# yongduosui/CAL

Measured on AMD Instinct MI355X. Metric: graphs/sec (train step) on SPMotif b=0.9 batch=128, higher is better.
Workload: dtype f32; 1 GPU; spmotif_b0.9_causalgcn_h128_l3_bs128; model=CausalGCN, batch_per_gpu=128, global_batch=128, hidden=128, layers=3, node_num=7, launch=graph(8 steps per graph launch, remainder 3), parallelism=dp1, resident_batches=8

## Files before the change

### cal_amd/csrc/engine.hip

```cpp
#include <string.h>
#include <hip/hip_ext.h>

#include <algorithm>
#include <type_traits>
#include <vector>

#include "engine_kernels.hpp"
#include "engine_readout.hpp"
#include "engine_gconv.hpp"
#include "engine_gconv_bwd.hpp"
#include "engine_ggat.hpp"
#include "engine_plan.hpp"
#include "engine_attbwd.hpp"
#include "engine_ro_step.hpp"
#include "engine_gin.hpp"
#include "engine_ggin.hpp"
#include "engine_feat.hpp"
#include "engine_gwide.hpp"
#include "engine_attwide.hpp"

extern "C" int cal_launch_gconv_bwd_att(unsigned gx, unsigned gy, hipStream_t st, hipEvent_t e0, hipEvent_t e1, const void* csr, size_t csr_bytes,
                                        const int* gptr, const int* eptr, const void* branches, size_t branches_bytes, float loop_w, int N, int H,
                                        int K, int* status, const void* att, size_t att_bytes);

namespace cal {

constexpr int MAX_LAYERS = 6;
constexpr int MAX_SLABS = 24;
constexpr int MAX_COMMITS = 64;

struct FinishArgs {
    SlabTask st[MAX_SLABS];
    CommitTask ct[MAX_COMMITS];
    int nst, nct;
    float* stats;
    float wc, wo, wco;
    float* tick;
    float* ticked;
    unsigned long long* perm_ctr;
    AdamArgs adam;
    AdamRange ar[MAX_ADAM_RANGES];
    int nar;
    double* bn0z; int bn0z_n;
    int* dirty;
    int* host_status;
    const int* status;
    int blk0[MAX_SLABS + MAX_COMMITS + MAX_ADAM_RANGES + 1];
};
__global__ void __launch_bounds__(256) k_finish(const FinishArgs fa, float* __restrict__ grad) {
    int task = 0;
    const int ntask = fa.nst + fa.nct + fa.nar;
    AdamArgs A = fa.adam;
    float adam_t = 0.f, adam_lr = 0.f;
    const bool flagged = fa.status && (fa.status[0] | fa.status[1]) != 0;
    if (fa.ticked && flagged && blockIdx.x == 0 && threadIdx.x == 0) fa.ticked[0] -= 1.f;
    if (A.on && flagged) A.on = 0;
    if (A.on) { adam_t = A.step[0]; adam_lr = A.lr[0]; }
    while (task + 1 < ntask && (int)blockIdx.x >= fa.blk0[task + 1]) ++task;
    const int bx = blockIdx.x - fa.blk0[task], nbx = fa.blk0[task + 1] - fa.blk0[task];
    if (fa.stats && blockIdx.x == 0 && threadIdx.x == 0)
        fa.stats[0] = fa.wc * fa.stats[1] + fa.wo * fa.stats[2] + fa.wco * fa.stats[3];
    if (fa.tick && !flagged && blockIdx.x == 0 && threadIdx.x == 0) fa.tick[0] += 1.f;
    if (fa.perm_ctr && blockIdx.x == 0 && threadIdx.x == 0) fa.perm_ctr[0] += 1;
    if (fa.bn0z && blockIdx.x == 0) {
        for (int i = threadIdx.x; i < fa.bn0z_n; i += 256) fa.bn0z[i] = 0.0;
        if (threadIdx.x == 0) *fa.dirty = 0;
    }
    if (fa.host_status && fa.status && blockIdx.x == 0 && threadIdx.x == 0)
        __hip_atomic_store(fa.host_status, fa.status[0] | fa.status[1], __ATOMIC_RELAXED, __HIP_MEMORY_SCOPE_SYSTEM);
    if (task < fa.nst) {
        const SlabTask t = fa.st[task];
        __shared__ float sred[256];
        const int el = threadIdx.x & 63, grp = threadIdx.x >> 6;
        const int per = (t.S + 3) / 4, z_lo = grp * per, z_hi = min(t.S, z_lo + per);
        for (int i0 = bx * 64; i0 < t.n; i0 += nbx * 64) {
            const int i = min(i0 + el, t.n - 1);
            float s0 = 0.f, s1 = 0.f;
            for (int z0 = z_lo; z0 < z_hi; z0 += 8) {
                float v[8];
#pragma unroll
                for (int u = 0; u < 8; ++u) v[u] = t.slabs[(size_t)max(min(z0 + u, z_hi - 1), 0) * t.n + i];
#pragma unroll
                for (int u = 0; u < 8; ++u) asm volatile("" : "+v"(v[u]));
#pragma unroll
                for (int u = 0; u < 8; u += 2) {
                    s0 += z0 + u < z_hi ? v[u] : 0.f;
                    s1 += z0 + u + 1 < z_hi ? v[u + 1] : 0.f;
                }
            }
            sred[threadIdx.x] = s0 + s1;
            __syncthreads();
            if (grp == 0 && i0 + el < t.n) {
                const float gsum = (sred[el] + sred[64 + el]) + (sred[128 + el] + sred[192 + el]);
                t.dst[i] = gsum;
                if (A.on) adam_update(A, (t.dst - grad) + i, gsum, adam_t, adam_lr);
            }
            __syncthreads();
        }
    } else if (task - fa.nst < fa.nct) {
        const CommitTask t = fa.ct[task - fa.nst];
        __shared__ double red[256];
        const int pl = threadIdx.x >> 4, cl = threadIdx.x & 15;
        for (int c0 = bx * 16; c0 < t.n; c0 += nbx * 16) {
            const int c = c0 + cl, cc = min(c, t.n - 1);
            double sacc = 0.0;
            for (int q0 = pl; q0 < t.P; q0 += 16 * 8) {
// ... 544 lines not shown
    }
    const dim3 grid(cdiv(N, rpb), nbranch);
    if (sd) {
        if (!wt || stt) { set_error("k_espmm: the fused SDDMM is built for the weighted branches without statistics"); return 2; }
        const bool pb = bb.b[0].pb_g != nullptr;
        if (pb != (bb.b[nbranch - 1].pb_g != nullptr)) { set_error("k_espmm: branches differ in kind"); return 2; }
        return with_g(H, [&](auto g) {
            constexpr int G = decltype(g)::value;
            if (pb) PROF_LAUNCH((k_espmm<4, G, true, false, true, true>), grid, dim3(256), 0, st, csr, bb, relu, loop_w, N, H, rpb);
            else PROF_LAUNCH((k_espmm<4, G, true, false, true>), grid, dim3(256), 0, st, csr, bb, relu, loop_w, N, H, rpb);
            return 0;
        });
    }
    return with_g(H, [&](auto g) {
        constexpr int G = decltype(g)::value;
        if (wt && stt) PROF_LAUNCH((k_espmm<4, G, true, true>), grid, dim3(256), 0, st, csr, bb, relu, loop_w, N, H, rpb);
        else if (wt) PROF_LAUNCH((k_espmm<4, G, true, false>), grid, dim3(256), 0, st, csr, bb, relu, loop_w, N, H, rpb);
        else if (stt) PROF_LAUNCH((k_espmm<4, G, false, true>), grid, dim3(256), 0, st, csr, bb, relu, loop_w, N, H, rpb);
        else PROF_LAUNCH((k_espmm<4, G, false, false>), grid, dim3(256), 0, st, csr, bb, relu, loop_w, N, H, rpb);
        return 0;
    });
}

Acc graph_acc(Ctx& c, double* dst, int cols, bool st = false) {
    if (st) return Acc(dst, nullptr, c.e->bn_plane);
    double* p = parts_alloc(c, (size_t)c.T * cols);
    if (!p) return Acc(dst);
    final_task(c, p, c.T, cols, cols, dst);
    return Acc(dst, p, cols);
}
CSR csr_dst(const Ctx& c) { return CSR{c.e->rowptr_dst, c.e->nbr_dst, c.e->eid_dst, (int)c.E}; }
CSR csr_src(const Ctx& c) { return CSR{c.e->rowptr_src, c.e->nbr_src, c.e->eid_src, (int)c.E}; }

template <typename Args>
int bn_bwd_sums(Ctx& c, Args& a, int P, double* dsum, double* dprod, bool st) {
    if (st) { a.dacc_sum = dsum; a.dacc_prod = dprod; a.dacc_ss = c.e->bn_plane; return 0; }
    const int H = c.e->H;
    double* p = parts_alloc(c, (size_t)P * 2 * H);
    if (!p) return no_parts();
    a.dot_parts = p;
    final_task(c, p, P, 2 * H, H, dsum);
    final_task(c, p + H, P, 2 * H, H, dprod);
    return 0;
}

int gconv_bwd(Ctx& c, Bwd& b, GconvBwdBranch* gb, int nb, float** dst, double** dsum, double** dprod, bool st, const AttBwdGraphArgs* att = nullptr) {
    Engine* e = c.e;
    const bool co = nb == 2;
    const bool wide = (co ? c.r.co_bwd : c.r.bb_bwd) == Conv::Wide;
    const int nsplit = co ? c.r.nsplit_co : c.r.nsplit_bb;
    const bool lean = co ? c.r.lean_co : c.r.lean_bb;
    const int H = e->H, B = c.T, nsl = H / GC_N;
    const int np2 = nsplit == 4 ? 2 : 1;
    for (int k = 0; k < nb; ++k) {
        gb[k].batch = c.batch; gb[k].tile_gptr = e->ntiles > 0 ? e->tile_gptr : nullptr;
        RCP(gb[k].slab = b.slabs(c, B, H * H, dst[k]));
        RC(bn_bwd_sums(c, gb[k], B * nsl * np2, dsum[k], dprod[k], st));
    }
    const GconvBwdBranch2 b2{{gb[0], gb[nb - 1]}};
    if (wide) {
        const CSR gs = csr_src(c);
        const dim3 gridw(B, nsl * nsplit, nb);
        if (co) PROF_LAUNCH((k_gw_bwd<true, 2>), gridw, dim3(GW_NT), 0, c.st, gs, e->gptr, e->eptr, b2, e->loop_w, c.N, H, H, nsplit, e->status);
        else if (gb[0].dout) PROF_LAUNCH((k_gw_bwd<false, 0>), gridw, dim3(GW_NT), 0, c.st, gs, e->gptr, e->eptr, b2, e->loop_w, c.N, H, H, nsplit, e->status);
        else PROF_LAUNCH((k_gw_bwd<false, 1>), gridw, dim3(GW_NT), 0, c.st, gs, e->gptr, e->eptr, b2, e->loop_w, c.N, H, H, nsplit, e->status);
        CAL_CHECK_LAUNCH("k_gw_bwd");
        return 0;
    }
    const CSR gd = csr_dst(c);
    const dim3 grid(B, nsl, nb);
    if (att) {
        if (co || lean || gb[0].dout) { set_error("k_gconv_bwd: the ATT mode is a one-branch, one-workgroup-per-CU launch"); return 2; }
        if (cal_launch_gconv_bwd_att(grid.x, grid.y, c.st, g_prof_cur ? g_prof_cur->r.e0 : nullptr, g_prof_cur ? g_prof_cur->r.e1 : nullptr, &gd, sizeof(gd),
                                     e->gptr, e->eptr, &b2, sizeof(b2), e->loop_w, c.N, H, H, e->status, att, sizeof(*att))) {
            set_error("k_gconv_bwd_att: argument structures differ between engine.hip and gconv_bwd_att.hip"); return 2;
        }
        if (g_prof_cur) g_prof_cur->used = true;
        CAL_CHECK_LAUNCH("k_att_bwd_graph");
        return 0;
    }
    const bool tiles = e->ntiles > 0;
    auto kern = co ? (lean ? (tiles ? k_gconv_bwd<true, 2, true, true> : k_gconv_bwd<true, 2, false, true>) : tiles ? k_gconv_bwd<true, 2, true> : k_gconv_bwd<true, 2>)
              : gb[0].dout ? (lean ? k_gconv_bwd<false, 0, false, true> : k_gconv_bwd<false, 0>) : lean ? k_gconv_bwd<false, 1, false, true> : k_gconv_bwd<false, 1>;
    PROF_LAUNCH(kern, grid, dim3(GB_NT), 0, c.st, gd, e->gptr, e->eptr, b2, e->loop_w, c.N, H, H, e->status);
    CAL_CHECK_LAUNCH("k_gconv_bwd");
    return 0;
}

RoArgs make_ro(const Ctx& c) {
    Engine* e = c.e;
    const int L = e->L, H = e->H, C = e->C, B = c.B;
    RoArgs a;
    memset(&a, 0, sizeof(a));
    for (int hd = 0; hd < 3; ++hd) {
        RoHead& h = a.h[hd];
        const int k1 = L + 3 + 2 * hd, k2 = L + 4 + 2 * hd;
        h.W1 = e->P + e->o_fc1_w[hd]; h.b1 = e->P + e->o_fc1_b[hd];
        h.W2 = e->P + e->o_fc2_w[hd]; h.b2 = e->P + e->o_fc2_b[hd];
        h.bn1 = bnref(c, k1, B, 1); h.bn2 = bnref(c, k2, B, 1);
        h.st2_sum = bn_stsum(c, k2); h.st2_sq = bn_stsq(c, k2);
        h.d1_sum = bn_dsum(c, k1); h.d1_prod = bn_dprod(c, k1);
        h.d2_sum = bn_dsum(c, k2); h.d2_prod = bn_dprod(c, k2);
        h.db1 = e->arena + e->a_db1 + hd * H; h.db2 = e->arena + e->a_db2 + hd * C;
        h.gW1 = e->G + e->o_fc1_w[hd]; h.gW2 = e->G + e->o_fc2_w[hd];
    }
    a.pooled = e->pooled; a.perm = c.perm; a.iperm = e->iperm; a.xco = e->xco; a.y1 = e->y1;
    a.zl = e->zl; a.logp = e->logp; a.dzl = e->dzl; a.dy1 = e->dy1; a.dxin = e->dxh;
    a.rowloss = e->dyh1;
    a.y = c.y; a.stats = e->stats; a.B = B; a.H = H; a.C = C;
    a.wc = c.wc; a.wo = c.wo; a.wco = c.wco; a.training = c.training; a.want_grad = c.want_grad;
    return a;
}

static int g_stop_after = 0;
static int g_stage = 0;
static std::vector<const char*> g_stage_names;
#define STAGE() do { if (g_stop_after == 0) g_stage_names.push_back(cal::g_last_launch); \
                     if (g_stop_after > 0 && ++g_stage >= g_stop_after) return -12345; } while (0)

int gin_rows(Ctx& c, int mode, const GinRowArgs& ga) {
    const int N = c.N, H = c.e->H;
    hipStream_t st = c.st;
    return with_g(H, [&](auto g) {
        constexpr int G = decltype(g)::value;
        const dim3 grid(cdiv(N, c.rpb_n));
        if (mode == 0) hipLaunchKernelGGL((k_gin_rows<4, G, 0>), grid, dim3(256), 0, st, ga, N, H, c.rpb_n);
        else if (mode == 1) hipLaunchKernelGGL((k_gin_rows<4, G, 1>), grid, dim3(256), 0, st, ga, N, H, c.rpb_n);
        else if (mode == 2) hipLaunchKernelGGL((k_gin_rows<4, G, 2>), grid, dim3(256), 0, st, ga, N, H, c.rpb_n);
        else hipLaunchKernelGGL((k_gin_rows<4, G, 3>), grid, dim3(256), 0, st, ga, N, H, c.rpb_n);
        return 0;
    });
}

template <typename Fn>
int with_g_fp(int H, int F, Fn f) {
    return with_g(H, [&](auto g) {
        constexpr int G = decltype(g)::value;
        if constexpr (G >= FEAT_FMAX) {
            if (F <= 4) return f(g, std::integral_constant<int, 4>());
            if (F <= 8) return f(g, std::integral_constant<int, 8>());
            if (F <= 12) return f(g, std::integral_constant<int, 12>());
            return f(g, std::integral_constant<int, 16>());
        } else {
            set_error("feature row kernels: hidden width too small"); return 2;
        }
    });
}

int pool2_slices(int N, int B) { return std::max(1, std::min(32, N / std::max(1, B * 128))); }
int launch_pool2(hipStream_t st, const float* hc, const float* ho, const int* gptr, float* pooled, float* cnt, float* slices,
                 int N, int B, int H) {
    const int tc = std::min(256, pow2ceil(H / 4));
    const int S = pool2_slices(N, B);
    hipLaunchKernelGGL((k_pool2<4>), dim3(B, 2, S), dim3(256), 0, st, hc, ho, gptr, pooled, pooled + (size_t)B * H, H, tc, slices, cnt);
    CAL_CHECK_LAUNCH("k_pool2");
    if (S > 1) {
        hipLaunchKernelGGL(k_pool2_sum, dim3(cdiv(4 * (int64_t)B * H, 256)), dim3(256), 0, st, slices, S, 2 * (int64_t)B * H, pooled, cnt);
        CAL_CHECK_LAUNCH("k_pool2_sum");
    }
    return 0;
}
int launch_pool2(Ctx& c) {
    Engine* e = c.e;
    const size_t NH = (size_t)c.N * e->H;
    return launch_pool2(c.st, e->hco, e->hco + NH, e->gptr, e->pooled, e->pcnt, e->dZco, (int)c.N, (int)c.B, e->H);
}
// ... 1218 lines not shown
    CAL_REQUIRE(e != nullptr && max_nodes >= 0 && max_edges >= 0, "bad arguments");
    e->max_nodes = (int)std::min<int64_t>(max_nodes, 1 << 30);
    e->max_edges = (int)std::min<int64_t>(max_edges, 1 << 30);
    return 0;
}
CAL_EXPORT int cal_engine_set_graph_ptrs(void* h, const int64_t* node_ptr, const int64_t* edge_ptr) {
    Engine* e = (Engine*)h;
    CAL_REQUIRE(e != nullptr, "bad arguments");
    e->node_ptr = node_ptr; e->edge_ptr = edge_ptr;
    return 0;
}
CAL_EXPORT int cal_engine_set_tiles(void* h, const int64_t* tile_gptr, int64_t ntiles) {
    Engine* e = (Engine*)h;
    CAL_REQUIRE(e != nullptr && ntiles >= 0 && (ntiles == 0 || tile_gptr != nullptr), "bad arguments");
    e->tile_gptr = ntiles > 0 ? tile_gptr : nullptr; e->ntiles = (int)ntiles;
    return 0;
}
CAL_EXPORT int cal_engine_set_deterministic(void* h, int on) {
    Engine* e = (Engine*)h;
    CAL_REQUIRE(e != nullptr, "bad arguments");
    e->striped = on ? 0 : 1;
    return 0;
}
CAL_EXPORT int cal_engine_debug_stop(int k) { g_stop_after = k; return 0; }
CAL_EXPORT const char* cal_engine_stage_name(int k) {
    return k >= 1 && k <= (int)g_stage_names.size() ? g_stage_names[k - 1] : "";
}

CAL_EXPORT int cal_sparse_probe_espmm(const int64_t* iv, void* const* pv, const double* dv, void* stream_) {
    CAL_REQUIRE(iv && pv && dv, "description missing");
    const int64_t nnz = iv[0], nbranch = iv[1], N = iv[3], H = iv[4], rpb = iv[5];
    CAL_REQUIRE(nbranch == 1 || nbranch == 2, "one or two branches");
    CAL_REQUIRE(H % 4 == 0 && H >= 4 && H <= 256, "hidden must be a multiple of 4 in [4, 256]");
    CAL_REQUIRE(N >= 1 && N < (1ll << 31) && nnz >= 0 && nnz < (1ll << 31) && rpb >= 1 && rpb < (1ll << 31), "sizes out of range");
    CSR csr;
    csr.ptr = (const int*)pv[0]; csr.nbr = (const int*)pv[1]; csr.eid = (const int*)pv[2]; csr.nnz = (int)nnz;
    SpmmBranch2 bb;
    for (int b = 0; b < 2; ++b) {
        const int64_t* ib = iv + 6 + 2 * std::min<int64_t>(b, nbranch - 1);
        void* const* pb = pv + 3 + 14 * std::min<int64_t>(b, nbranch - 1);
        SpmmBranch& br = bb.b[b];
        br.h = (const float*)pb[0]; br.out = (float*)pb[1]; br.bias = (const float*)pb[2]; br.w = (const float*)pb[3];
        br.dis = (const float*)pb[4];
        br.st_sum = Acc((double*)pb[5], (double*)pb[6], (int)ib[0]);
        br.st_sq = Acc((double*)pb[7], (double*)pb[8], (int)ib[1]);
        br.sd_z = (const float*)pb[9]; br.sd_gn = (float*)pb[10]; br.sd_gself = (float*)pb[11];
        br.pb_g = (const float*)pb[12]; br.pb_batch = (const int64_t*)pb[13];
    }
    RC(launch_espmm((hipStream_t)stream_, csr, bb, (int)nbranch, (int)iv[2], (float)dv[0], (int)N, (int)H, (int)rpb));
    CAL_CHECK_LAUNCH("k_espmm(probe)");
    return 0;
}
CAL_EXPORT int cal_sparse_probe_edge_att(const int* ptr, const int* nbr, const int* eid, int64_t nnz, const float* pq, const float* be,
                                         float* att, float* dis_c, float* dis_o, double loop_w, int64_t N, int64_t E, double fedge,
                                         void* stream_) {
    CAL_REQUIRE(ptr && nbr && eid && pq && be && att && dis_c && dis_o, "null argument");
    CAL_REQUIRE(N >= 1 && N < (1ll << 31) && E >= 0 && nnz >= 0 && nnz < (1ll << 31), "sizes out of range");
    CSR gs;
    gs.ptr = ptr; gs.nbr = nbr; gs.eid = eid; gs.nnz = (int)nnz;
    hipLaunchKernelGGL(k_edge_att_deg, dim3(cdiv(N, 32)), dim3(256), 0, (hipStream_t)stream_, gs, pq, be, att, dis_c, dis_o,
                       (float)loop_w, (int)N, E, (float)fedge);
    CAL_CHECK_LAUNCH("k_edge_att_deg(probe)");
    return 0;
}
CAL_EXPORT int cal_sparse_probe_pool(int sel, const float* hc, const float* ho, const int* gptr, const int64_t* batch, float* pooled,
                                     float* cnt, float* slices, int64_t N, int64_t B, int64_t H, int64_t rpb_n, int64_t* S_out,
                                     void* stream_) {
    CAL_REQUIRE(sel >= 0 && sel <= 3 && S_out != nullptr, "bad selector");
    CAL_REQUIRE(H % 4 == 0 && H >= 4 && H <= 256, "hidden must be a multiple of 4 in [4, 256]");
    CAL_REQUIRE(N >= 1 && N < (1ll << 31) && B >= 1 && B < (1ll << 31), "sizes out of range");
    const int S = pool2_slices((int)N, (int)B);
    *S_out = S;
    if (sel == 3) return 0;
    CAL_REQUIRE(hc && ho && (sel == 2 ? batch != nullptr && cnt != nullptr && rpb_n >= 1 && rpb_n < (1ll << 31) : gptr != nullptr && pooled != nullptr),
                "null argument");
    if (sel == 2) return launch_pool_cnt((hipStream_t)stream_, hc, ho, batch, cnt, (int)N, (int)B, (int)H, (int)rpb_n);
    CAL_REQUIRE(S == 1 || slices != nullptr, "row slices without a slice buffer");
    return launch_pool2((hipStream_t)stream_, hc, ho, gptr, pooled, sel == 0 ? cnt : nullptr, slices, (int)N, (int)B, (int)H);
}
#ifdef CAL_BLK_CLOCKS
CAL_EXPORT int cal_debug_blk_clocks(long long* out) {
    return (int)hipMemcpyFromSymbol(out, HIP_SYMBOL(cal::g_blk_clk), sizeof(long long) * 8192);
}
#endif
#ifdef CAL_RO_CLOCKS
CAL_EXPORT int cal_debug_ro_clocks(long long* out) {
    return (int)hipMemcpyFromSymbol(out, HIP_SYMBOL(cal::g_ro_clk), sizeof(long long) * 64);
}
#endif

CAL_EXPORT int cal_engine_profile(int on) {
    g_prof_on = on != 0;
    if (on) {
        for (auto& r : g_prof) { hipEventDestroy(r.e0); hipEventDestroy(r.e1); }
        g_prof.clear();
    }
    return 0;
}
CAL_EXPORT int64_t cal_engine_profile_read(double* out, int64_t cap) {
    int64_t n = 0;
    for (auto& r : g_prof) {
        if (n >= cap) break;
        float ms = 0.f;
        if (hipEventElapsedTime(&ms, r.e0, r.e1) != hipSuccess) ms = -1.f;
        out[3 * n] = r.cls; out[3 * n + 1] = ms; out[3 * n + 2] = r.work;
        ++n;
    }
    return n;
}

CAL_EXPORT int cal_engine_adam(void* h, void* stream_) {
    Engine* e = (Engine*)h;
    hipStream_t st = (hipStream_t)stream_;
    RC(launch_adam(e, st, 0));
    hipLaunchKernelGGL(k_adam_tick, dim3(1), dim3(1), 0, st, e->step);
    CAL_CHECK_LAUNCH("k_adam_tick");
    return 0;
}
CAL_EXPORT int cal_engine_adam_ticked(void* h, void* stream_) {
    return launch_adam((Engine*)h, (hipStream_t)stream_, 1);
}
CAL_EXPORT int cal_p2p_alloc(int64_t bytes, void** out) {
    CAL_REQUIRE(bytes > 0 && out, "bad arguments");
    void* p = nullptr;
    hipError_t rc = hipExtMallocWithFlags(&p, (size_t)bytes, hipDeviceMallocFinegrained);
    if (rc != hipSuccess || !p) { (void)hipGetLastError(); set_error("cal_p2p_alloc: hipExtMallocWithFlags(fine-grained, %lld bytes): %s", (long long)bytes, hipGetErrorString(rc)); return 3; }
    rc = hipMemset(p, 0, (size_t)bytes);
    if (rc == hipSuccess) rc = hipDeviceSynchronize();
    if (rc != hipSuccess) { (void)hipGetLastError(); (void)hipFree(p); set_error("cal_p2p_alloc: zeroing failed: %s", hipGetErrorString(rc)); return 3; }
    *out = p;
    return 0;
}
CAL_EXPORT int cal_p2p_free(void* p) {
    if (p && hipFree(p) != hipSuccess) { (void)hipGetLastError(); set_error("cal_p2p_free failed"); return 3; }
    return 0;
}
CAL_EXPORT int cal_p2p_export(void* p, void* handle64) {
    CAL_REQUIRE(p && handle64, "bad arguments");
    static_assert(sizeof(hipIpcMemHandle_t) == 64, "IPC handle size");
    hipIpcMemHandle_t hd;
    hipError_t rc = hipIpcGetMemHandle(&hd, p);
    if (rc != hipSuccess) { (void)hipGetLastError(); set_error("cal_p2p_export: hipIpcGetMemHandle: %s", hipGetErrorString(rc)); return 3; }
    memcpy(handle64, &hd, 64);
    return 0;
}
CAL_EXPORT int cal_p2p_open(const void* handle64, void** out) {
    CAL_REQUIRE(handle64 && out, "bad arguments");
    hipIpcMemHandle_t hd;
    memcpy(&hd, handle64, 64);
    void* p = nullptr;
    hipError_t rc = hipIpcOpenMemHandle(&p, hd, hipIpcMemLazyEnablePeerAccess);
    if (rc != hipSuccess || !p) { (void)hipGetLastError(); set_error("cal_p2p_open: hipIpcOpenMemHandle: %s", hipGetErrorString(rc)); return 3; }
    *out = p;
    return 0;
}
CAL_EXPORT int cal_p2p_close(void* p) {
    if (p && hipIpcCloseMemHandle(p) != hipSuccess) { (void)hipGetLastError(); set_error("cal_p2p_close failed"); return 3; }
    return 0;
}
CAL_EXPORT int64_t cal_engine_p2p_region_bytes(void* h) {
    Engine* e = (Engine*)h;
    const int64_t np = (e->nparam + 63) / 64 * 64;
    return (2 * np + 64) * 4;
}
CAL_EXPORT int cal_engine_p2p_bind(void* h, void* const* peer_bases, const int64_t* peer_devices, int64_t world, int64_t rank) {
    Engine* e = (Engine*)h;
// ... 79 lines not shown
```

### cal_amd/csrc/engine_gconv_bwd.hpp

```cpp
#pragma once
#include "engine_gconv.hpp"
#include "engine_attphases.hpp"

namespace cal {

constexpr int GB_NT = 512;
constexpr int GB_T = 64;
constexpr int GB_E = 1024;
constexpr int GB_LDJ = GB_T + 1;
constexpr int GB_LDD = GC_N + 4;
constexpr int GB_LDW = GC_K + 1;
constexpr int GB_LDX = GC_K + 4;

struct GconvBwdBranch {
    const float* dout;
    const float* x;
    const float* W;
    const float* ew;
    const float* dis;
    const float* rs;
    int rs_stride;
    BNRef bn;
    float* dxp0; float* dxp1;
    float* slab;
    double* dot_parts;
    double* dacc_sum; double* dacc_prod; int dacc_ss;
    const float* coef_in;
    const float* dy0; const float* dy1;
    const float* y;
    BNRef ubn;
    const double* udot_sum; const double* udot_prod;
    double* bias_parts;
    const float* gp0; const float* gp1; const int* iperm;
    const float* z;
    float* gn; float* gself;
    size_t gn_stride, gself_stride;
    int gn_slot;
    const int64_t* batch;
    const int64_t* tile_gptr;
};

struct GconvBwdBranch2 { GconvBwdBranch b[2]; };
struct GconvBwdNoAtt {};
template <int MODE> struct GconvBwdNoAttOf { using type = GconvBwdNoAtt; };

template <bool RS, int MODE, bool TILED = false, bool LEAN = false>
__global__ void __launch_bounds__(GB_NT, (LEAN ? 4 : 1)) k_gconv_bwd(const CSR g, const int* __restrict__ gptr, const int* __restrict__ eptr,
                                                   const GconvBwdBranch2 bb, float loop_w, int N, int H,
                                                   int K, int* __restrict__ status) {
    static_assert(MODE != 3, "the ATT mode is the kernel k_gconv_bwd_att (gconv_bwd_att.hip)");
    [[maybe_unused]] const typename GconvBwdNoAttOf<MODE>::type ga{};
#include "engine_gconv_bwd_body.hpp"
}

constexpr int FB_T = 64, FB_F = 64, FB_H = 128;
struct FeatBwdArgs {
    const float* dy0; const float* dy1;
    const float* y;
    BNRef ubn; const double* udot_sum; const double* udot_prod;
    const float* x0;
    const float* W;
    BNRef bn0;
    float* slab;
    double* parts;
};
template <int FMAX>
__global__ void __launch_bounds__(GB_NT) k_feat_bwd(const int* __restrict__ gptr, const FeatBwdArgs a, int H, int F,
                                                  int* __restrict__ status, int N) {
    __shared__ __attribute__((aligned(16))) float Dz[FB_T * (FB_H + 4)];
    __shared__ float Xn[FB_T * FMAX];
    __shared__ __attribute__((aligned(16))) float Ws[FMAX * (FB_H + 4)];
    __shared__ float um_s[FB_H], ur_s[FB_H], ug_s[FB_H], u1_s[FB_H], u2_s[FB_H];
    __shared__ float m0_s[FMAX], r0_s[FMAX], g0_s[FMAX], b0_s[FMAX];
    __shared__ float dX0[FB_T * FMAX];
    BLK_CLK(0);
    warm_kernargs<sizeof(FeatBwdArgs) + 32>();
    const int b = blockIdx.x, t = threadIdx.x, LDZ = FB_H + 4;
    const int g0 = gptr ? gptr[b] : b * FB_T, rows = gptr ? gptr[b + 1] - g0 : min(FB_T, N - g0);
    float* slab = a.slab + (size_t)b * F * H;
    double* parts = a.parts + (size_t)b * 2 * F;
    if (rows <= 0 || rows > FB_T) {
        if (rows > 0 && t == 0) atomicOr(status, 8);
        for (int i = t; i < F * H; i += GB_NT) slab[i] = 0.f;
        for (int i = t; i < 2 * F; i += GB_NT) parts[i] = 0.0;
        return;
    }
    const int H4 = H >> 2;
// ... 300 lines not shown
```

### cal_amd/csrc/engine_gconv_bwd_body.hpp

```cpp
    constexpr int LDX = LEAN ? GC_K : GB_LDX;
    __shared__ __attribute__((aligned(16))) float Ab[GB_T * GB_LDJ];
    __shared__ __attribute__((aligned(16))) float Ds[GB_T * GB_LDD];
    __shared__ __attribute__((aligned(16))) float Ws[LEAN ? 4 : GC_K * GB_LDD];
    __shared__ __attribute__((aligned(16))) float Xs[GB_T * LDX];
    __shared__ float mean_s[GC_K], rstd_s[GC_K], gam_s[GC_K], bet_s[GC_K];
    __shared__ int ptr_s[GB_T + 4];
    __shared__ float dis_s[GB_T], rs_s[GB_T];
    __shared__ unsigned char en[GB_E];
    __shared__ float ec[GB_E];
    __shared__ float um_s[MODE == 1 ? GC_N : 1], ur_s[MODE == 1 ? GC_N : 1], ug_s[MODE == 1 ? GC_N : 1], u1_s[MODE == 1 ? GC_N : 1], u2_s[MODE == 1 ? GC_N : 1];
    __shared__ float bs_s[GB_NT / 64][16][4];
    __shared__ __attribute__((aligned(16))) float Zr_own[(MODE == 2 && !LEAN) ? GB_T * GB_LDD : 4];
    float* const Zr = (MODE == 2 && LEAN) ? Xs : Zr_own;
    __shared__ float gv_s[TILED ? GC_TILE_GRAPHS * GC_N : GC_N];
    __shared__ unsigned char bg_s[TILED ? GB_T : 4];
    __shared__ int ee[(MODE == 2 && !LEAN) ? GB_E : 1];
    __shared__ unsigned char er[GB_E];
    constexpr bool UP = MODE == 1, POOL = MODE == 2, ATT = MODE == 3;
    static_assert(!TILED || MODE == 2, "only the POOL variant looks at the graphs inside a tile");
    static_assert(!ATT || (!LEAN && !RS), "the ATT mode keeps the staged W slice (one workgroup per CU) and has no row scales");
    __shared__ double red[ATT ? 8 : 1][4][ATT ? GC_N : 1];
    __shared__ double sc_lds[2][ATT ? 8 : 1];
    __shared__ float bnk_s[ATT ? 8 : 1][ATT ? GC_K : 1];
    __shared__ float dis_c_s[ATT ? GB_T : 1], dis_o_s[ATT ? GB_T : 1], dd_c_s[ATT ? GB_T : 1], dd_o_s[ATT ? GB_T : 1], spv_s[ATT ? GB_T : 1], sqv_s[ATT ? GB_T : 1],
// ... 281 lines not shown
        float cs[4] = {0.f, 0.f, 0.f, 0.f};
        const bool two = br.dy1 != nullptr;
#pragma unroll
        for (int u = 0; u < 2; ++u) { ro_pin(bd.v[u]); ro_pin(bd1.v[u]); ro_pin(by.v[u]); }
        const int c = 4 * (t & 15);
#pragma unroll
        for (int u = 0; u < 2; ++u) {
            const int j = (t >> 4) + u * (GB_NT / 16);
            if (j < rows) {
                const float4 v0 = bd.v[u], v1 = bd1.v[u], yv = by.v[u];
                const float d[4] = {v0.x + (two ? v1.x : 0.f), v0.y + (two ? v1.y : 0.f), v0.z + (two ? v1.z : 0.f), v0.w + (two ? v1.w : 0.f)};
                const float yy[4] = {yv.x, yv.y, yv.z, yv.w};
                float o[4];
#pragma unroll
                for (int q = 0; q < 4; ++q) {
                    const float yn = (yy[q] - um_s[c + q]) * ur_s[c + q];
                    const float g1 = ug_s[c + q] * (d[q] - u1_s[c + q] - yn * u2_s[c + q]);
                    o[q] = yy[q] > 0.f ? g1 : 0.f;
                    cs[q] += o[q];
                }
                *reinterpret_cast<float4*>(Ds + j * GB_LDD + c) = make_float4(o[0], o[1], o[2], o[3]);
            }
        }
#pragma unroll
        for (int q = 0; q < 4; ++q) {
            cs[q] += __shfl_xor(cs[q], 16, 64);
            cs[q] += __shfl_xor(cs[q], 32, 64);
        }
        if (lane < 16) {
#pragma unroll
            for (int q = 0; q < 4; ++q) bs_s[t >> 6][lane][q] = cs[q];
        }
    }
    for (int i = t; i < (rowsP - rows) * GB_LDD; i += GB_NT) Ds[rows * GB_LDD + i] = 0.f;
    for (int i = t; i < (rowsP - rows) * LDX; i += GB_NT) Xs[rows * LDX + i] = 0.f;
    if (!ATT) adj_scatter<GB_NT, GB_LDJ>(Ab, er, en, un, t, [&](int j, int s) { return dis_s[j] * ec[s]; }, [&](int j) { return dis_s[j] * dis_s[j] * loop_w; });
    __syncthreads();
    if ((UP || POOL) && t < GC_N) {
        double tot = 0.0;
#pragma unroll
        for (int k = 0; k < GB_NT / 64; ++k) tot += (double)bs_s[k][t >> 2][t & 3];
        br.bias_parts[(size_t)b * H + ns0 + t] = tot;
    }
    if (!ATT) BLK_CLK(2); else BLK_CLK_W(3, 0, t);
    auto ident = [](float v) { return v; };
    gc_f32x16 acc[2];
    {
        const int rt = w >> 1, ct = w & 1;
#pragma unroll
        for (int i = 0; i < 16; ++i) { acc[0][i] = 0.f; acc[1][i] = 0.f; }
        if (rt < R) mma_kmajor<1, 1, GB_LDJ, GB_LDD>(Ab + rt * 32 + li, Ds + ct * 32 + li, rowsP, lk, ident, MmaIdent(), acc);
        if constexpr (ATT) { if (w >= 4) att_colsum_store(ga.a, red, sc_lds, t - 256, 256, ns0, GC_N, H, sl == 0); }
        if (POOL && w >= 4) {
            const int q4 = (t - 256) & 3, it0 = (t - 256) >> 2;
            float* gn = br.gn + (size_t)sl * br.gn_stride;
            float* gs = br.gself + (size_t)sl * br.gself_stride;
            for (int it = it0; it - it0 < ne + rows; it += 64) {
                const bool ok = it < ne + rows, isedge = it < ne;
                const int itc = ok ? it : 0;
                const int jd = isedge ? er[itc] : itc - ne, js = isedge ? en[itc] : itc - ne;
                const float4* a = reinterpret_cast<const float4*>(Ds + (ok ? jd : 0) * GB_LDD + 16 * q4);
                const float4* bsrc = reinterpret_cast<const float4*>(Zr + (ok ? js : 0) * GB_LDD + 16 * q4);
                float p = 0.f;
#pragma unroll
                for (int k = 0; k < 4; ++k) p = dot4(a[k], bsrc[k], p);
                p += __shfl_xor(p, 1, 64);
                p += __shfl_xor(p, 2, 64);
                if (ok && q4 == 0) {
                    if (isedge) gn[(LEAN || br.gn_slot) ? e0 + itc : ee[itc]] = p; else gs[g0 + itc - ne] = p;
                }
            }
        }
        __syncthreads();
        if (POOL && LEAN) commit_x();
        if (rt < R) {
#pragma unroll
            for (int r = 0; r < 16; ++r) {
                const int row = mma_row(r, lk, rt * 32);
                Ds[row * GB_LDD + ct * 32 + li] = acc[0][r];
            }
        }
        __syncthreads();
    }
    if (w < 4 && w * 32 < K) {
#pragma unroll
        for (int i = 0; i < 16; ++i) { acc[0][i] = 0.f; acc[1][i] = 0.f; }
        const float* wrow = LEAN ? br.W + (size_t)min(w * 32 + li, K - 1) * H + ns0 : Ws + (w * 32 + li) * GB_LDD;
        if (R == 2) mma_rowk<true>(Ds + li * GB_LDD, Ds + (32 + li) * GB_LDD, wrow, GC_N, lk, acc[0], acc[1]);
        else mma_rowk<false>(Ds + li * GB_LDD, nullptr, wrow, GC_N, lk, acc[0], acc[1]);
        const int k = w * 32 + li;
        float* dxp = sl ? br.dxp1 : br.dxp0;
        float xh[2][16];
#pragma unroll
        for (int q = 0; q < 2; ++q)
#pragma unroll
            for (int r = 0; r < 16; ++r) xh[q][r] = Xs[(mma_row(r, lk, q * 32)) * LDX + k];
#pragma unroll
        for (int q = 0; q < 2; ++q)
#pragma unroll
            for (int r = 0; r < 16; ++r) { asm volatile("" : "+v"(xh[q][r])); if (q >= R) xh[q][r] = 0.f; }
        float f1[4] = {0.f, 0.f, 0.f, 0.f}, f2[4] = {0.f, 0.f, 0.f, 0.f};
#pragma unroll
        for (int q = 0; q < 2; ++q) {
#pragma unroll
            for (int r = 0; r < 16; ++r) {
                const int i = mma_row(r, lk, q * 32);
                const float v = acc[q][r];
                f1[r & 3] += v;
                f2[r & 3] = fmaf(v, xh[q][r], f2[r & 3]);
            }
        }
        gc_store_tile<gc_site(WT_DXP)>(acc[0], dxp + (size_t)g0 * K + w * 32, K, rows, li, lk, MmaIdent(), (rows * K - w * 32) * 4);
        if (R == 2) gc_store_tile<gc_site(WT_DXP)>(acc[1], dxp + (size_t)(g0 + 32) * K + w * 32, K, rows - 32, li, lk, MmaIdent(), ((rows - 32) * K - w * 32) * 4);
        double s1, s2;
        colsum_fold(f1, f2, s1, s2);
        if (lk == 0) {
            if (br.dacc_sum) {
                const size_t po = (size_t)stripe_of_block() * br.dacc_ss + k;
                atomicAdd(br.dacc_sum + po, s1); atomicAdd(br.dacc_prod + po, s2);
            } else { parts[k] = s1; parts[K + k] = s2; }
        }
    }
    if (!ATT) BLK_CLK(3);
    if (w >= 4 && (w - 4) * 32 < K) {
        const int wq = w - 4, k = wq * 32 + li;
        const float gam = gam_s[k], bet = bet_s[k];
        auto affine = [&](float v) { return fmaf(v, gam, bet); };
#pragma unroll
        for (int i = 0; i < 16; ++i) { acc[0][i] = 0.f; acc[1][i] = 0.f; }
        mma_kmajor<1, 2, LDX, GB_LDD>(Xs + wq * 32 + li, Ds + li, rowsP, lk, affine, MmaIdent(), acc);
#pragma unroll
        for (int q = 0; q < 2; ++q) {
            const int off = wq * 32 * H + ns0 + q * 32;
            gc_store_tile<gc_site(WT_DW)>(acc[q], slab + off, H, 32, li, lk, MmaIdent(), (K * H - off) * 4);
        }
    }
    BLK_CLK(1);
```

### cal_amd/csrc/engine_kernels.hpp

```cpp
#pragma once
#include "engine.hpp"

namespace cal {

#ifdef CAL_BLK_CLOCKS
__device__ long long g_blk_clk[4 * 2048];
#define BLK_CLK(which) do { const int b_ = blockIdx.x + gridDim.x * blockIdx.y; \
                            if (threadIdx.x == 0 && b_ < 2048) g_blk_clk[4 * b_ + ((which) == 1 ? 3 : (which) == 0 ? 0 : (which) - 1)] = wall_clock64(); } while (0)
#define BLK_CLK_W(which, wv, dep) do { const int b_ = blockIdx.x + gridDim.x * blockIdx.y; int d_; \
                            asm volatile("s_waitcnt vmcnt(0) lgkmcnt(0)\n\tv_readfirstlane_b32 %0, %1" : "=s"(d_) : "v"(dep)); \
                            if ((int)threadIdx.x == 64 * (wv) && b_ < 2048) g_blk_clk[4 * b_ + ((which) == 1 ? 3 : (which) == 0 ? 0 : (which) - 1)] = wall_clock64() + (d_ & 0); } while (0)
#else
#define BLK_CLK(which) do {} while (0)
#define BLK_CLK_W(which, wv, dep) do {} while (0)
#endif

struct CSR {
    const int* ptr;
    const int* nbr;
    const int* eid;
    int nnz;
};

struct Acc {
    double* dst;
    double* parts;
    int stride;
    __host__ __device__ Acc() : dst(nullptr), parts(nullptr), stride(0) {}
    __host__ __device__ Acc(double* d) : dst(d), parts(nullptr), stride(0) {}
    __host__ __device__ Acc(double* d, double* p, int s) : dst(d), parts(p), stride(s) {}
    __host__ __device__ bool on() const { return dst != nullptr || parts != nullptr; }
    __device__ __forceinline__ void add(int col, double t) const {
        if (parts) parts[(size_t)blockIdx.x * stride + col] = t;
        else atomicAdd(dst + (size_t)stripe_of_block() * stride + col, t);
    }
};

__device__ __forceinline__ void block_col_atomic(double v, int cslot, int rlane, int nrl, int ncols, bool valid,
                                                 const Acc& dst, int col, double* lds) {
    lds[rlane * ncols + cslot] = valid ? v : 0.0;
    __syncthreads();
    if (rlane == 0 && valid) {
        double t = 0.0;
        for (int k = 0; k < nrl; ++k) t += lds[k * ncols + cslot];
        dst.add(col, t);
    }
    __syncthreads();
}

template <int NV>
__device__ __forceinline__ void block_col_sums(const double (&v)[NV], int cslot, int rlane, int nrl, int ncols, bool valid,
                                               double* lds, double (&out)[NV]) {
#pragma unroll
    for (int q = 0; q < NV; ++q) lds[(q * nrl + rlane) * ncols + cslot] = valid ? v[q] : 0.0;
    __syncthreads();
    if (rlane == 0 && valid) {
#pragma unroll
        for (int q = 0; q < NV; ++q) {
            double t = 0.0;
            for (int k = 0; k < nrl; ++k) t += lds[(q * nrl + k) * ncols + cslot];
            out[q] = t;
        }
    }
    __syncthreads();
}

struct FinalTask { const double* parts; int P; int stride; int n; double* dst; };
struct FinalArgs { FinalTask t[8]; int nt; };
__global__ void __launch_bounds__(256) k_stats_final(const FinalArgs fa) {
    __shared__ double red[256];
    const FinalTask t = fa.t[blockIdx.y];
    const int c = blockIdx.x * 8 + (threadIdx.x & 7), pl = threadIdx.x >> 3;
    const int cc = min(c, t.n - 1);
    double s0 = 0.0, s1 = 0.0;
    for (int p0 = pl; p0 < t.P; p0 += 32 * 8) {
        double v[8];
#pragma unroll
        for (int u = 0; u < 8; ++u) v[u] = t.parts[(size_t)min(p0 + 32 * u, t.P - 1) * t.stride + cc];
#pragma unroll
        for (int u = 0; u < 8; ++u) asm volatile("" : "+v"(v[u]));
#pragma unroll
        for (int u = 0; u < 8; u += 2) {
            s0 += p0 + 32 * u < t.P ? v[u] : 0.0;
            s1 += p0 + 32 * (u + 1) < t.P ? v[u + 1] : 0.0;
        }
    }
    red[threadIdx.x] = s0 + s1;
    __syncthreads();
    if (pl == 0 && c < t.n) {
        double tot = 0.0;
#pragma unroll
        for (int k = 0; k < 32; ++k) tot += red[k * 8 + (threadIdx.x & 7)];
        t.dst[c] = tot;
    }
}

constexpr int ZP_CAP = 1024;
// ... 1168 lines not shown
```

### cal_amd/csrc/gconv_bwd_att.hip

```cpp
#include <hip/hip_runtime.h>
#include <hip/hip_ext.h>
#include <stdint.h>
#include <string.h>

namespace {
#include "engine_kernels.hpp"
#include "engine_readout.hpp"
#include "engine_gconv.hpp"
#include "engine_gconv_bwd.hpp"
#include "engine_attbwd.hpp"

namespace cal {
__global__ void __launch_bounds__(GB_NT, 1) k_gconv_bwd_att(const CSR g, const int* __restrict__ gptr, const int* __restrict__ eptr,
                                                           const GconvBwdBranch2 bb, float loop_w, int N, int H,
                                                           int K, int* __restrict__ status, const AttBwdGraphArgs ga) {
    constexpr bool RS = false, TILED = false, LEAN = false;
    constexpr int MODE = 3;
#include "engine_gconv_bwd_body.hpp"
}
}
}

extern "C" int cal_launch_gconv_bwd_att(unsigned gx, unsigned gy, hipStream_t st, hipEvent_t e0, hipEvent_t e1, const void* csr, size_t csr_bytes,
                                        const int* gptr, const int* eptr, const void* branches, size_t branches_bytes, float loop_w, int N, int H,
                                        int K, int* status, const void* att, size_t att_bytes) {
    using namespace cal;
    if (csr_bytes != sizeof(CSR) || branches_bytes != sizeof(GconvBwdBranch2) || att_bytes != sizeof(AttBwdGraphArgs)) return 2;
    CSR g; GconvBwdBranch2 bb; AttBwdGraphArgs ga;
    memcpy(&g, csr, sizeof(g)); memcpy(&bb, branches, sizeof(bb)); memcpy(&ga, att, sizeof(ga));
    const dim3 grid(gx, gy, 1);
    if (e0) hipExtLaunchKernelGGL(k_gconv_bwd_att, grid, dim3(GB_NT), 0, st, e0, e1, 0, g, gptr, eptr, bb, loop_w, N, H, K, status, ga);
    else hipLaunchKernelGGL(k_gconv_bwd_att, grid, dim3(GB_NT), 0, st, g, gptr, eptr, bb, loop_w, N, H, K, status, ga);
    return 0;
}
```

Before: 619,500 graphs/s.

## Split gconv backward dX work across all waves and run dW after

Adds a sequential variant of the gconv backward tail. All eight waves now compute the dX tiles, each wave taking one row tile and one 32-column slice, and the two row-tile halves of the column sums are combined through LDS. The dW tiles are then computed in a second phase, replacing the old split where waves 0-3 did dX and waves 4-7 did dW concurrently. The variant is compiled in a separate translation unit and selected by default (CAL_GCB_ORDER=1) for the non-lean instantiations. It also adds extra clock instrumentation macros for timing each phase.

```diff
diff --git a/cal_amd/csrc/engine.hip b/cal_amd/csrc/engine.hip
--- a/cal_amd/csrc/engine.hip
+++ b/cal_amd/csrc/engine.hip
@@ -22,6 +22,9 @@
 extern "C" int cal_launch_gconv_bwd_att(unsigned gx, unsigned gy, hipStream_t st, hipEvent_t e0, hipEvent_t e1, const void* csr, size_t csr_bytes,
                                         const int* gptr, const int* eptr, const void* branches, size_t branches_bytes, float loop_w, int N, int H,
                                         int K, int* status, const void* att, size_t att_bytes);
+extern "C" int cal_launch_gconv_bwd_seq(int sel, unsigned gx, unsigned gy, unsigned gz, hipStream_t st, hipEvent_t e0, hipEvent_t e1, const void* csr,
+                                        size_t csr_bytes, const int* gptr, const int* eptr, const void* branches, size_t branches_bytes, float loop_w,
+                                        int N, int H, int K, int* status);
 
 namespace cal {
 
@@ -732,6 +735,15 @@
     const bool tiles = e->ntiles > 0;
     auto kern = co ? (lean ? (tiles ? k_gconv_bwd<true, 2, true, true> : k_gconv_bwd<true, 2, false, true>) : tiles ? k_gconv_bwd<true, 2, true> : k_gconv_bwd<true, 2>)
               : gb[0].dout ? (lean ? k_gconv_bwd<false, 0, false, true> : k_gconv_bwd<false, 0>) : lean ? k_gconv_bwd<false, 1, false, true> : k_gconv_bwd<false, 1>;
+    if (CAL_GCB_ORDER != 0 && (!lean || CAL_GCB_ORDER == 2)) {
+        const int sel = (co ? 1 : 0) | (co && tiles ? 2 : 0) | (!co && gb[0].dout ? 4 : 0) | (lean ? 8 : 0);
+        const int rc = cal_launch_gconv_bwd_seq(sel, grid.x, grid.y, grid.z, c.st, g_prof_cur ? g_prof_cur->r.e0 : nullptr, g_prof_cur ? g_prof_cur->r.e1 : nullptr,
+                                                &gd, sizeof(gd), e->gptr, e->eptr, &b2, sizeof(b2), e->loop_w, c.N, H, H, e->status);
+        if (rc) { set_error(rc == 2 ? "k_gconv_bwd: argument structures differ between engine.hip and gconv_bwd_seq.hip" : "k_gconv_bwd: instantiation missing from gconv_bwd_seq.hip"); return 2; }
+        if (g_prof_cur) g_prof_cur->used = true;
+        CAL_CHECK_LAUNCH("k_gconv_bwd");
+        return 0;
+    }
     PROF_LAUNCH(kern, grid, dim3(GB_NT), 0, c.st, gd, e->gptr, e->eptr, b2, e->loop_w, c.N, H, H, e->status);
     CAL_CHECK_LAUNCH("k_gconv_bwd");
     return 0;
@@ -2116,6 +2128,9 @@
 CAL_EXPORT int cal_debug_blk_clocks(long long* out) {
     return (int)hipMemcpyFromSymbol(out, HIP_SYMBOL(cal::g_blk_clk), sizeof(long long) * 8192);
 }
+CAL_EXPORT int cal_debug_blk_clocks_x(long long* out) {
+    return (int)hipMemcpyFromSymbol(out, HIP_SYMBOL(cal::g_blk_clk_x), sizeof(long long) * 8192);
+}
 #endif
 #ifdef CAL_RO_CLOCKS
 CAL_EXPORT int cal_debug_ro_clocks(long long* out) {
diff --git a/cal_amd/csrc/engine_gconv_bwd.hpp b/cal_amd/csrc/engine_gconv_bwd.hpp
--- a/cal_amd/csrc/engine_gconv_bwd.hpp
+++ b/cal_amd/csrc/engine_gconv_bwd.hpp
@@ -3,6 +3,15 @@
 #include "engine_attphases.hpp"
 
 namespace cal {
+
+#ifndef CAL_GCB_ORDER
+#define CAL_GCB_ORDER 1
+#endif
+#ifdef CAL_GCB_UNIT
+constexpr bool GCB_SEQ = CAL_GCB_ORDER != 0, GCB_SEQ_LEAN = CAL_GCB_ORDER == 2;
+#else
+constexpr bool GCB_SEQ = false, GCB_SEQ_LEAN = false;
+#endif
 
 constexpr int GB_NT = 512;
 constexpr int GB_T = 64;
diff --git a/cal_amd/csrc/engine_gconv_bwd_body.hpp b/cal_amd/csrc/engine_gconv_bwd_body.hpp
--- a/cal_amd/csrc/engine_gconv_bwd_body.hpp
+++ b/cal_amd/csrc/engine_gconv_bwd_body.hpp
@@ -387,12 +387,72 @@
         }
         __syncthreads();
     }
+    constexpr bool SEQ = GCB_SEQ && (!LEAN || GCB_SEQ_LEAN);
+    if constexpr (SEQ) {
+    {
+        const int rt = w >> 2, kq = w & 3, k = kq * 32 + li;
+        const bool on = kq * 32 < K;
+        float4* const park = reinterpret_cast<float4*>(Ab);
+        float xh[16];
+        float f1[4] = {0.f, 0.f, 0.f, 0.f}, f2[4] = {0.f, 0.f, 0.f, 0.f};
+#pragma unroll
+        for (int i = 0; i < 16; ++i) acc[0][i] = 0.f;
+        if (on) {
+            const float* wrow = LEAN ? br.W + (size_t)k * H + ns0 : Ws + k * GB_LDD;
+            if (rt < R) mma_rowk(Ds + (rt * 32 + li) * GB_LDD, wrow, GC_N, lk, acc[0]);
+            BLK_CLK_X(4, 4, acc[0][15]);
+#pragma unroll
+            for (int r = 0; r < 16; ++r) xh[r] = Xs[(mma_row(r, lk, rt * 32)) * LDX + k];
+#pragma unroll
+            for (int r = 0; r < 16; ++r) { asm volatile("" : "+v"(xh[r])); if (rt >= R) xh[r] = 0.f; }
+            float* dxp = sl ? br.dxp1 : br.dxp0;
+            if (rt < R) gc_store_tile<gc_site(WT_DXP)>(acc[0], dxp + (size_t)(g0 + rt * 32) * K + kq * 32, K, rows - rt * 32, li, lk, MmaIdent(),
+                                                       ((rows - rt * 32) * K - kq * 32) * 4);
+            if (rt == 0) {
+#pragma unroll
+                for (int r = 0; r < 16; ++r) { const float v = acc[0][r]; f1[r & 3] += v; f2[r & 3] = fmaf(v, xh[r], f2[r & 3]); }
+                park[(2 * kq) * 64 + lane] = make_float4(f1[0], f1[1], f1[2], f1[3]);
+                park[(2 * kq + 1) * 64 + lane] = make_float4(f2[0], f2[1], f2[2], f2[3]);
+            }
+        }
+        __syncthreads();
+        if (!ATT) BLK_CLK(3);
+        if (on && rt == 1) {
+            const float4 p1 = park[(2 * kq) * 64 + lane], p2 = park[(2 * kq + 1) * 64 + lane];
+            f1[0] = p1.x; f1[1] = p1.y; f1[2] = p1.z; f1[3] = p1.w;
+            f2[0] = p2.x; f2[1] = p2.y; f2[2] = p2.z; f2[3] = p2.w;
+#pragma unroll
+            for (int r = 0; r < 16; ++r) { const float v = acc[0][r]; f1[r & 3] += v; f2[r & 3] = fmaf(v, xh[r], f2[r & 3]); }
+            double s1, s2;
+            colsum_fold(f1, f2, s1, s2);
+            if (lk == 0) {
+                if (br.dacc_sum) {
+                    const size_t po = (size_t)stripe_of_block() * br.dacc_ss + k;
+                    atomicAdd(br.dacc_sum + po, s1); atomicAdd(br.dacc_prod + po, s2);
+                } else { parts[k] = s1; parts[K + k] = s2; }
+            }
+        }
+        BLK_CLK_X(5, 4, f1[0]);
+    }
+    if (w < (K >> 4)) {
+        const int ct = w >= (K >> 5) ? 1 : 0, kt = w - ct * (K >> 5), k = kt * 32 + li;
+        const float gam = gam_s[k], bet = bet_s[k];
+        auto affine = [&](float v) { return fmaf(v, gam, bet); };
+#pragma unroll
+        for (int i = 0; i < 16; ++i) acc[0][i] = 0.f;
+        mma_kmajor_ptrs<1, 1, LDX, GB_LDD>(Xs + kt * 32 + li, nullptr, Ds + ct * 32 + li, nullptr, rowsP, lk, affine, MmaIdent(), acc);
+        const int off = kt * 32 * H + ns0 + ct * 32;
+        gc_store_tile<gc_site(WT_DW)>(acc[0], slab + off, H, 32, li, lk, MmaIdent(), (K * H - off) * 4);
+    }
+    BLK_CLK_X(6, 4, acc[0][15]);
+    } else {
     if (w < 4 && w * 32 < K) {
 #pragma unroll
         for (int i = 0; i < 16; ++i) { acc[0][i] = 0.f; acc[1][i] = 0.f; }
         const float* wrow = LEAN ? br.W + (size_t)min(w * 32 + li, K - 1) * H + ns0 : Ws + (w * 32 + li) * GB_LDD;
         if (R == 2) mma_rowk<true>(Ds + li * GB_LDD, Ds + (32 + li) * GB_LDD, wrow, GC_N, lk, acc[0], acc[1]);
         else mma_rowk<false>(Ds + li * GB_LDD, nullptr, wrow, GC_N, lk, acc[0], acc[1]);
+        BLK_CLK_X(4, 0, acc[0][15]);
         const int k = w * 32 + li;
         float* dxp = sl ? br.dxp1 : br.dxp0;
         float xh[2][16];
@@ -425,6 +485,7 @@
                 atomicAdd(br.dacc_sum + po, s1); atomicAdd(br.dacc_prod + po, s2);
             } else { parts[k] = s1; parts[K + k] = s2; }
         }
+        BLK_CLK_X(5, 0, f1[0]);
     }
     if (!ATT) BLK_CLK(3);
     if (w >= 4 && (w - 4) * 32 < K) {
@@ -439,5 +500,7 @@
             const int off = wq * 32 * H + ns0 + q * 32;
             gc_store_tile<gc_site(WT_DW)>(acc[q], slab + off, H, 32, li, lk, MmaIdent(), (K * H - off) * 4);
         }
+        BLK_CLK_X(6, 4, acc[1][15]);
+    }
     }
     BLK_CLK(1);
diff --git a/cal_amd/csrc/engine_kernels.hpp b/cal_amd/csrc/engine_kernels.hpp
--- a/cal_amd/csrc/engine_kernels.hpp
+++ b/cal_amd/csrc/engine_kernels.hpp
@@ -10,9 +10,15 @@
 #define BLK_CLK_W(which, wv, dep) do { const int b_ = blockIdx.x + gridDim.x * blockIdx.y; int d_; \
                             asm volatile("s_waitcnt vmcnt(0) lgkmcnt(0)\n\tv_readfirstlane_b32 %0, %1" : "=s"(d_) : "v"(dep)); \
                             if ((int)threadIdx.x == 64 * (wv) && b_ < 2048) g_blk_clk[4 * b_ + ((which) == 1 ? 3 : (which) == 0 ? 0 : (which) - 1)] = wall_clock64() + (d_ & 0); } while (0)
+__device__ long long g_blk_clk_x[4 * 2048];
+#define BLK_CLK_X(which, wv, dep) do { if (__builtin_amdgcn_readfirstlane((int)threadIdx.x >> 6) == (wv)) { \
+                            const int b_ = blockIdx.x + gridDim.x * blockIdx.y; int d_; \
+                            asm volatile("s_waitcnt vmcnt(0) lgkmcnt(0)\n\tv_readfirstlane_b32 %0, %1" : "=s"(d_) : "v"(dep)); \
+                            if ((int)threadIdx.x == 64 * (wv) && b_ < 2048) g_blk_clk_x[4 * b_ + (which) - 4] = wall_clock64() + (d_ & 0); } } while (0)
 #else
 #define BLK_CLK(which) do {} while (0)
 #define BLK_CLK_W(which, wv, dep) do {} while (0)
+#define BLK_CLK_X(which, wv, dep) do {} while (0)
 #endif
 
 struct CSR {
diff --git a/cal_amd/csrc/gconv_bwd_att.hip b/cal_amd/csrc/gconv_bwd_att.hip
--- a/cal_amd/csrc/gconv_bwd_att.hip
+++ b/cal_amd/csrc/gconv_bwd_att.hip
@@ -3,6 +3,7 @@
 #include <stdint.h>
 #include <string.h>
 
+#define CAL_GCB_UNIT
 namespace {
 #include "engine_kernels.hpp"
 #include "engine_readout.hpp"
@@ -33,3 +34,10 @@
     else hipLaunchKernelGGL(k_gconv_bwd_att, grid, dim3(GB_NT), 0, st, g, gptr, eptr, bb, loop_w, N, H, K, status, ga);
     return 0;
 }
+
+#ifdef CAL_BLK_CLOCKS
+extern "C" __attribute__((visibility("default"))) int cal_debug_blk_clocks_att(long long* out, long long* outx) {
+    const int rc = (int)hipMemcpyFromSymbol(out, HIP_SYMBOL(cal::g_blk_clk), sizeof(long long) * 8192);
+    return rc ? rc : (int)hipMemcpyFromSymbol(outx, HIP_SYMBOL(cal::g_blk_clk_x), sizeof(long long) * 8192);
+}
+#endif
diff --git a/cal_amd/csrc/gconv_bwd_seq.hip b/cal_amd/csrc/gconv_bwd_seq.hip
--- /dev/null
+++ b/cal_amd/csrc/gconv_bwd_seq.hip
@@ -0,0 +1,50 @@
+#include <hip/hip_runtime.h>
+#include <hip/hip_ext.h>
+#include <stdint.h>
+#include <string.h>
+
+#define CAL_GCB_UNIT
+namespace {
+#include "engine_kernels.hpp"
+#include "engine_readout.hpp"
+#include "engine_gconv.hpp"
+#include "engine_gconv_bwd.hpp"
+}
+
+extern "C" int cal_launch_gconv_bwd_seq(int sel, unsigned gx, unsigned gy, unsigned gz, hipStream_t st, hipEvent_t e0, hipEvent_t e1, const void* csr,
+                                        size_t csr_bytes, const int* gptr, const int* eptr, const void* branches, size_t branches_bytes, float loop_w,
+                                        int N, int H, int K, int* status) {
+    using namespace cal;
+    if (csr_bytes != sizeof(CSR) || branches_bytes != sizeof(GconvBwdBranch2)) return 2;
+#if CAL_GCB_ORDER == 0
+    return 3;
+#else
+    CSR g; GconvBwdBranch2 bb;
+    memcpy(&g, csr, sizeof(g)); memcpy(&bb, branches, sizeof(bb));
+    void (*kern)(const CSR, const int*, const int*, const GconvBwdBranch2, float, int, int, int, int*) = nullptr;
+    switch (sel) {
+        case 1: kern = k_gconv_bwd<true, 2>; break;
+        case 3: kern = k_gconv_bwd<true, 2, true>; break;
+        case 4: kern = k_gconv_bwd<false, 0>; break;
+        case 0: kern = k_gconv_bwd<false, 1>; break;
+#if CAL_GCB_ORDER == 2
+        case 9: kern = k_gconv_bwd<true, 2, false, true>; break;
+        case 11: kern = k_gconv_bwd<true, 2, true, true>; break;
+        case 12: kern = k_gconv_bwd<false, 0, false, true>; break;
+        case 8: kern = k_gconv_bwd<false, 1, false, true>; break;
+#endif
+        default: return 3;
+    }
+    const dim3 grid(gx, gy, gz);
+    if (e0) hipExtLaunchKernelGGL(kern, grid, dim3(GB_NT), 0, st, e0, e1, 0, g, gptr, eptr, bb, loop_w, N, H, K, status);
+    else hipLaunchKernelGGL(kern, grid, dim3(GB_NT), 0, st, g, gptr, eptr, bb, loop_w, N, H, K, status);
+    return 0;
+#endif
+}
+
+#ifdef CAL_BLK_CLOCKS
+extern "C" __attribute__((visibility("default"))) int cal_debug_blk_clocks_seq(long long* out, long long* outx) {
+    const int rc = (int)hipMemcpyFromSymbol(out, HIP_SYMBOL(cal::g_blk_clk), sizeof(long long) * 8192);
+    return rc ? rc : (int)hipMemcpyFromSymbol(outx, HIP_SYMBOL(cal::g_blk_clk_x), sizeof(long long) * 8192);
+}
+#endif
```

New measurement: 628,000 graphs/s, median of 6. 1.01x the previous value.
